# grasingerm/polymer-stats

Hardware: NVIDIA B200
Metric: monomer MC updates/sec (whole box), interacting n=512 dielectric chains (higher is better)
Workload: dtype f64

## Files before the change

polymer-stats_b200/csrc/cta_kernels.cuh:

```cuda
#pragma once

#include <type_traits>

#include "chain_math.cuh"

namespace pmc {

constexpr int kPartDoubles = 96;
constexpr int kRowDoubles = 26;

struct CtaView {
  double *sx, *sy, *sz;
  double *mx, *my, *mz;
  double *E;
  double *part;
  double *rowbuf;
  Proposal* prop;
  ChainDyn* dyn;
  ChainParams* par;
};

__host__ __device__ inline size_t cta_smem_bytes(int n) {
  size_t b = (size_t)7 * n * sizeof(double);
  b += (kPartDoubles + kRowDoubles) * sizeof(double);
// ... 101 lines not shown
    S.mx[i] = ux; S.my[i] = uy; S.mz[i] = uz;
  }
  team_sync<T>();
}

template <int T>
__device__ double cta_pair_energy(const CtaView& S, int n, int energy_type, double crad2 = 0.0) {
  constexpr int W = T / 32;
  const int tid = threadIdx.x, lane = tid & 31, warp = tid >> 5;
  double acc = 0.0;
  if (energy_type == 3) {
    for (int i = warp; i < n - 1; i += W) {
      const double xi = S.sx[i], yi = S.sy[i], zi = S.sz[i];
      const double ax = S.mx[i], ay = S.my[i], az = S.mz[i];
      for (int j = i + 1 + lane; j < n; j += 32)
        acc += pair_g_cut(ax, ay, az, S.mx[j], S.my[j], S.mz[j], xi - S.sx[j], yi - S.sy[j], zi - S.sz[j], crad2);
    }
  } else if (energy_type == 1) {
    for (int i = warp; i < n - 1; i += W) {
      const double xi = S.sx[i], yi = S.sy[i], zi = S.sz[i];
      const double ax = S.mx[i], ay = S.my[i], az = S.mz[i];
      for (int j = i + 1 + lane; j < n; j += 32)
        acc += pair_g(ax, ay, az, S.mx[j], S.my[j], S.mz[j], xi - S.sx[j], yi - S.sy[j], zi - S.sz[j]);
    }
  } else if (energy_type == 2) {
    for (int i = tid; i < n - 1; i += T)
      acc += pair_g(S.mx[i], S.my[i], S.mz[i], S.mx[i + 1], S.my[i + 1], S.mz[i + 1],
                    S.sx[i] - S.sx[i + 1], S.sy[i] - S.sy[i + 1], S.sz[i] - S.sz[i + 1]);
  }
  return block_sum<T>(acc, S.part);
}

template <int NW>
struct Team {
  static constexpr int kWarps = NW;
  static constexpr int kThreads = NW * 32;
  static constexpr int kLocalThreads = NW * 32;
  __device__ __forceinline__ static int tid() { return (int)threadIdx.x; }
  __device__ __forceinline__ static int ltid() { return tid(); }
  __device__ __forceinline__ static int warp() { return (int)(threadIdx.x >> 5); }
  __device__ __forceinline__ static int lane() { return (int)(threadIdx.x & 31); }
  __device__ __forceinline__ static void sync() { __syncthreads(); }
};

struct WarpTeam {
  static constexpr int kWarps = 1;
  static constexpr int kThreads = 32;
  static constexpr int kLocalThreads = 32;
  __device__ __forceinline__ static int tid() { return (int)(threadIdx.x & 31); }
  __device__ __forceinline__ static int ltid() { return tid(); }
  __device__ __forceinline__ static int warp() { return 0; }
  __device__ __forceinline__ static int lane() { return (int)(threadIdx.x & 31); }
  __device__ __forceinline__ static void sync() { __syncwarp(); }
};

struct LaneItem {
  double x, y, z;
  double ax, ay, az;
  double tx, ty, tz;
  double c;
  double w;
};

__device__ __forceinline__ LaneItem load_lane_item(const CtaView& S, int L, double Dx, double Dy, double Dz) {
  LaneItem it;
  it.x = S.sx[L]; it.y = S.sy[L]; it.z = S.sz[L];
  it.ax = S.mx[L]; it.ay = S.my[L]; it.az = S.mz[L];
  it.tx = -3.0 * it.ax; it.ty = -3.0 * it.ay; it.tz = -3.0 * it.az;
  it.c = fma(it.tz, Dz, fma(it.ty, Dy, it.tx * Dx));
  it.w = 0.0;
  return it;
}

__device__ __forceinline__ double rect_proj(double x, double y, double z, double px, double py, double pz, double Dx,
                                            double Dy, double Dz) {
  return fma(z - pz, Dz, fma(y - py, Dy, (x - px) * Dx));
}

__device__ __forceinline__ void rect_lane_w(LaneItem& it, double px, double py, double pz, double Dx, double Dy,
                                            double Dz) {
  it.w = -2.0 * rect_proj(it.x, it.y, it.z, px, py, pz, Dx, Dy, Dz);
}

template <bool Q2>
__device__ __forceinline__ void rect_prepass_item(const CtaView& S, int baseB, int k, double px, double py, double pz,
                                                  double Dx, double Dy, double Dz) {
  const int j = baseB + k;
  const double e = fma(S.mz[j], Dz, fma(S.my[j], Dy, S.mx[j] * Dx));
  if constexpr (Q2) {
    const double dd = fma(Dz, Dz, fma(Dy, Dy, Dx * Dx));
    reinterpret_cast<double2*>(S.E)[k] =
        make_double2(e, fma(2.0, rect_proj(S.sx[j], S.sy[j], S.sz[j], px, py, pz, Dx, Dy, Dz), dd));
  }
  else
    S.E[j] = e;
}

template <bool CUT = false, bool Q2 = false>
__device__ __forceinline__ double rect_pair(const LaneItem& it, double bx, double by, double bz, double ux,
                                            double uy, double uz, double e, double p2, double Dx, double Dy, double Dz,
                                            double acc, double crad2 = 0.0) {
  const double rx = it.x - bx, ry = it.y - by, rz = it.z - bz;
  const double mm = fma(it.az, uz, fma(it.ay, uy, it.ax * ux));
  const double r2 = fma(rz, rz, fma(ry, ry, rx * rx));
  const double a3 = fma(it.tz, rz, fma(it.ty, ry, it.tx * rx));
  const double bb = fma(uz, rz, fma(uy, ry, ux * rx));
  double q2;
  if constexpr (Q2) {
    q2 = (r2 + it.w) + p2;
  } else {
    const double qx = rx - Dx, qy = ry - Dy, qz = rz - Dz;
    q2 = fma(qz, qz, fma(qy, qy, qx * qx));
  }
  const double a3n = a3 - it.c;
  const double bn = bb - e;
  const double y = rsqrt_fast(r2);
  const double yn = rsqrt_fast(q2);
  const double y2 = y * y, yn2 = yn * yn;
  const double t = fma(a3 * bb, y2, mm);
  const double tn = fma(a3n * bn, yn2, mm);
  if constexpr (CUT) {
    const double gn = tn * (yn2 * yn), go = t * (y2 * y);
    return acc + ((q2 > crad2 ? 0.0 : gn) - (r2 > crad2 ? 0.0 : go));
  } else {
    acc = fma(tn, yn2 * yn, acc);
    return fma(-t, y2 * y, acc);
  }
}

template <class TEAM, int UNROLL = 2, bool CUT = false, bool EFLY = false, bool Q2 = false>
__device__ __forceinline__ double rect_sum(const CtaView& S, int baseA, int A, int baseB, int B, double Dx,
                                           double Dy, double Dz, double crad2 = 0.0, int pivot = 0) {
  static_assert(!(Q2 && EFLY), "the Q2 form reads 2p_B from the pre-pass");
  constexpr int W = TEAM::kWarps;
  const int lane = TEAM::lane(), warp = TEAM::warp();
  const int G = (A + 31) >> 5;
  const double* __restrict__ bxp = S.sx + baseB;
  const double* __restrict__ byp = S.sy + baseB;
  const double* __restrict__ bzp = S.sz + baseB;
  const double* __restrict__ mxp = S.mx + baseB;
  const double* __restrict__ myp = S.my + baseB;
  const double* __restrict__ mzp = S.mz + baseB;
  const double* __restrict__ ep = S.E + baseB;
  const double2* __restrict__ e2p = reinterpret_cast<const double2*>(S.E);
  auto lane_item = [&](int L) {
    LaneItem it = load_lane_item(S, L, Dx, Dy, Dz);
    if (Q2) {
      rect_lane_w(it, S.sx[pivot], S.sy[pivot], S.sz[pivot], Dx, Dy, Dz);
      asm("" : "+d"(it.tx), "+d"(it.ty), "+d"(it.tz));
    }
    return it;
  };
  auto bvals = [&](int k, double ux, double uy, double uz, double& e, double& p2) {
    if constexpr (Q2) {
      const double2 v = e2p[k];
      e = v.x; p2 = v.y;
    } else {
      e = EFLY ? fma(uz, Dz, fma(uy, Dy, ux * Dx)) : ep[k];
      p2 = 0.0;
    }
  };
  double acc = 0.0;
  const int G2 = G >> 1;
  {
    const int U = G2 * B;
    int u = (int)(((long long)U * warp) / W);
    const int u1 = (int)(((long long)U * (warp + 1)) / W);
    if (u < u1) {
      int g = u / B;
      int k = u - g * B;
      while (u < u1) {
        const int l0 = g * 64 + lane, l1 = l0 + 32;
        const bool v0 = l0 < A, v1 = l1 < A;
        const LaneItem i0 = lane_item(baseA + min(l0, A - 1));
        const LaneItem i1 = lane_item(baseA + min(l1, A - 1));
        const int kend = min(B, k + (u1 - u));
        u += kend - k;
        double a0 = 0.0, a1 = 0.0;
#pragma unroll UNROLL
        for (; k < kend; ++k) {
          const double bx = bxp[k], by = byp[k], bz = bzp[k];
          const double ux = mxp[k], uy = myp[k], uz = mzp[k];
          double e, p2;
          bvals(k, ux, uy, uz, e, p2);
          a0 = rect_pair<CUT, Q2>(i0, bx, by, bz, ux, uy, uz, e, p2, Dx, Dy, Dz, a0, crad2);
          a1 = rect_pair<CUT, Q2>(i1, bx, by, bz, ux, uy, uz, e, p2, Dx, Dy, Dz, a1, crad2);
        }
        acc += (v0 ? a0 : 0.0) + (v1 ? a1 : 0.0);
        k = 0;
        ++g;
      }
    }
  }
  if (G & 1) {
    int k = (int)(((long long)B * warp) / W);
    const int kend = (int)(((long long)B * (warp + 1)) / W);
    if (k < kend) {
      const int li = (G - 1) * 32 + lane;
      const bool valid = li < A;
      const LaneItem it = lane_item(baseA + min(li, A - 1));
      double a0 = 0.0, a1 = 0.0;
      auto pair = [&](int kk, double a) {
        double e, p2;
        bvals(kk, mxp[kk], myp[kk], mzp[kk], e, p2);
        return rect_pair<CUT, Q2>(it, bxp[kk], byp[kk], bzp[kk], mxp[kk], myp[kk], mzp[kk], e, p2, Dx, Dy, Dz, a,
                                  crad2);
      };
      for (; k + 1 < kend; k += 2) {
        a0 = pair(k, a0);
        a1 = pair(k + 1, a1);
      }
      if (k < kend) a0 = pair(k, a0);
      acc += valid ? (a0 + a1) : 0.0;
    }
  }
  return acc;
}

template <class TEAM, int UNROLL = 2>
__device__ __forceinline__ double delta_pairs_partial(const CtaView& S, int n, int energy_type, double b, int idx,
                                                      double npx, double npy, double npz,
                                                      double dnx, double dny, double dnz) {
  constexpr int T = TEAM::kThreads;
  const int tid = TEAM::tid();
  const double Dx = b * dnx, Dy = b * dny, Dz = b * dnz;
  const double hx = 0.5 * Dx, hy = 0.5 * Dy, hz = 0.5 * Dz;
  const int H = idx, Tl = n - 1 - idx;
  bool rect = (energy_type == 1) && H > 0 && Tl > 0;
  bool lanes_are_heads = true;
  if (rect) {
    const long long costH = (long long)((H + 31) >> 5) * Tl;
    const long long costT = (long long)((Tl + 31) >> 5) * H;
    lanes_are_heads = costH <= costT;
    if (2 * (lanes_are_heads ? Tl : H) > n) lanes_are_heads = !lanes_are_heads;
  }
  const double sgn = lanes_are_heads ? 1.0 : -1.0;
  const double ex = sgn * Dx, ey = sgn * Dy, ez = sgn * Dz;
  const int baseA = lanes_are_heads ? 0 : idx + 1, A = lanes_are_heads ? H : Tl;
  const int baseB = lanes_are_heads ? idx + 1 : 0, B = lanes_are_heads ? Tl : H;
  const double xi = S.sx[idx], yi = S.sy[idx], zi = S.sz[idx];
  if (rect)
    for (int k = TEAM::ltid(); k < B; k += TEAM::kLocalThreads)
      rect_prepass_item<true>(S, baseB, k, xi, yi, zi, ex, ey, ez);
  double acc = 0.0;
  {
    const double ox = S.mx[idx], oy = S.my[idx], oz = S.mz[idx];
    int jlo = 0, jhi = n - 1;
    if (energy_type == 2) { jlo = max(0, idx - 1); jhi = min(n - 1, idx + 1); }
    if (energy_type == 0) { jlo = 1; jhi = 0; }
    for (int j = jlo + tid; j <= jhi; j += T) {
      if (j == idx) continue;
      const double rx = xi - S.sx[j], ry = yi - S.sy[j], rz = zi - S.sz[j];
      const double s = (j < idx) ? 1.0 : -1.0;
      const double ux = S.mx[j], uy = S.my[j], uz = S.mz[j];
      acc += pair_g(npx, npy, npz, ux, uy, uz, fma(s, hx, rx), fma(s, hy, ry), fma(s, hz, rz)) -
             pair_g(ox, oy, oz, ux, uy, uz, rx, ry, rz);
    }
  }
  TEAM::sync();
  if (rect) acc += rect_sum<TEAM, UNROLL, false, false, true>(S, baseA, A, baseB, B, ex, ey, ez, 0.0, idx);
  return acc;
}

template <int T, int UNROLL = 2>
__device__ __forceinline__ double cta_delta_pairs(const CtaView& S, int n, int energy_type, double b, int idx,
                                                  double npx, double npy, double npz, double dnx, double dny,
                                                  double dnz) {
  const double acc = delta_pairs_partial<Team<T / 32>, UNROLL>(S, n, energy_type, b, idx, npx, npy, npz, dnx, dny, dnz);
  return block_sum<T>(acc, S.part, false);
}

}

#define PMC_CTA_BUILDING_BLOCKS 1
#include "cta_f32.cuh"

namespace pmc {

struct RunArgs {
  MonoRec* mono;
  const ChainParams* par;
  ChainDyn* dyn;
  double* traj;
  double* roll;
  long long nsteps, stepout, rows;
  uint64_t seed;
  uint32_t chain_id_base;
  int n;
  int nchains;
  int energy_type;
  ChainDynX* dynx;
  double* state;
  int roll_cols;
  int compensated;
  int window;
};

__device__ __forceinline__ void make_proposal(const RunArgs& a, const ChainParams& P, const ChainDyn& D,
                                              const MonoRec* mono, uint32_t chain_id, uint32_t init, long long step,
                                              Proposal& q) {
  const Draws d = draw_step(a.seed, chain_id, init, step, a.n);
  const MonoRec rec = mono[d.idx];
  double dphi, dtheta;
  increments(P, d, rec.theta, D.phi_step, D.theta_step, dphi, dtheta);
  build_proposal(P, rec, d.idx, dphi, dtheta, d.eps, q);
}

__device__ __forceinline__ void apply_decision(const ChainParams& P, ChainDyn& D, const Proposal& q, bool accept,
                                               double dU_pairs, long long step) {
  if (accept) {
    D.U += q.du + q.drF + dU_pairs;
    D.Omega += q.dOmega;
    D.su += q.du;
    D.r[0] += P.b * q.dnx; D.r[1] += P.b * q.dny; D.r[2] += P.b * q.dnz;
    D.p[0] += q.dmx; D.p[1] += q.dmy; D.p[2] += q.dmz;
    D.nacc += 1;
    D.nacc_total += 1;
  }
  D.natt += 1;
  D.steps_total += 1;
  D.step = step;
}

template <bool COMP = true>
__device__ __forceinline__ void bookkeep(const ChainParams& P, ChainDyn& D, long long step) {
  adapt_steps(P, step, D.phi_step, D.theta_step, D.nacc, D.natt);
  record_averages<COMP>(P, D.acc, D.comp, D.r, D.p, D.U, D.su, D.log_gauge);
}

template <bool COMP = true>
__device__ __forceinline__ void after_decision(const ChainParams& P, ChainDyn& D, const Proposal& q, bool accept,
                                               double dU_pairs, long long step) {
  apply_decision(P, D, q, accept, dU_pairs, step);
  bookkeep<COMP>(P, D, step);
}

__device__ __forceinline__ void stage_row(const ChainDyn& D, long long step, double* rowbuf) {
  rowbuf[0] = (double)step;
  rowbuf[1] = D.r[0]; rowbuf[2] = D.r[1]; rowbuf[3] = D.r[2];
  rowbuf[4] = D.p[0]; rowbuf[5] = D.p[1]; rowbuf[6] = D.p[2];
  rowbuf[7] = D.U;
  rowbuf[8] = (double)step;
  const double nrm = D.acc[16] + D.comp[16];
#pragma unroll
  for (int k = 0; k < 16; ++k) rowbuf[9 + k] = (D.acc[k] + D.comp[k]) / nrm;
}

__device__ __forceinline__ void emit_row(const RunArgs& a, const ChainDyn& D, int c, long long row, long long step,
                                         double* rowbuf, int tid) {
  if (tid == 0) stage_row(D, step, rowbuf);
  __syncwarp();
  if (row < a.rows) {
    if (tid < 8) a.traj[((size_t)c * a.rows + row) * 8 + tid] = rowbuf[tid];
    if (tid < 17) a.roll[((size_t)c * a.rows + row) * 17 + tid] = rowbuf[8 + tid];
  }
  __syncwarp();
}

__device__ __forceinline__ MonoRec record_of(const Proposal& q) {
  MonoRec rec;
  rec.phi = q.phi; rec.theta = q.theta;
  rec.nx = q.nx; rec.ny = q.ny; rec.nz = q.nz; rec.sth = q.sth;
  return rec;
}

__device__ __forceinline__ void shift_tail(const CtaView& S, int first, int n, double Dx, double Dy, double Dz, int tid,
                                           int stride) {
  for (int j = first + tid; j < n; j += stride) {
    S.sx[j] += Dx; S.sy[j] += Dy; S.sz[j] += Dz;
  }
}

__device__ __forceinline__ void move_pivot(const CtaView& S, MonoRec* mono, const Proposal& q, int idx, double b,
                                           double dnx, double dny, double dnz) {
  S.sx[idx] += 0.5 * b * dnx; S.sy[idx] += 0.5 * b * dny; S.sz[idx] += 0.5 * b * dnz;
  S.mx[idx] = q.mx; S.my[idx] = q.my; S.mz[idx] = q.mz;
  mono[idx] = record_of(q);
}

__device__ __forceinline__ bool decide(double single, double tsum, double inv_kT, double eps, double& dsum) {
  dsum = __dmul_rn(kInv4Pi, tsum);
  return metropolis(__fma_rn(-dsum, inv_kT, single), eps);
}

constexpr int kWin = 32;

__device__ __forceinline__ int window_len(const RunArgs& a, const ChainParams& P, bool adapt_on, long long step0,
                                          long long s, long long& to_boundary) {
  long long wl = a.nsteps - s + 1;
  if (wl > kWin) wl = kWin;
  to_boundary = 0;
  if (adapt_on) {
    to_boundary = P.steps_per_adjust - ((step0 + s - 1) % P.steps_per_adjust);
    if (wl > to_boundary) wl = to_boundary;
  }
  return (int)wl;
}

template <class Make>
__device__ __forceinline__ void build_window(long long step, int wlen, unsigned& dirty, int tid, Make&& make) {
  if (tid < wlen) make(tid, step + tid);
  if (tid == 0) dirty = 0u;
}

template <class Entry>
__device__ __forceinline__ void mark_stale(const Entry* win, int k, int wlen, int lo, int hi, unsigned& dirty,
                                           int tid) {
  const int widx = win[tid].idx;
  const bool stale = tid > k && tid < wlen && widx >= lo && widx <= hi;
  const unsigned m = __ballot_sync(0xffffffffu, stale);
  if (tid == 0 && m) dirty |= m;
}

__host__ __device__ inline size_t cta_smem_bytes_win(int n) {
  return (cta_smem_bytes(n) + kWin * sizeof(Proposal) + 16 + 15) & ~(size_t)15;
}
__host__ __device__ inline size_t cta_smem_bytes_win_f32(int n) { return cta_smem_bytes_win(n) + f32_smem_bytes(n); }

template <int T, int MINB, int UNROLL = 2, int PREC = 0>
__global__ void __launch_bounds__(T, MINB) k_run_cta_win(const RunArgs a) {
  extern __shared__ __align__(16) unsigned char smem_raw[];
  const CtaView S = carve(smem_raw, a.n);
  Proposal* win = reinterpret_cast<Proposal*>(smem_raw + cta_smem_bytes(a.n));
  unsigned* dirty = reinterpret_cast<unsigned*>(win + kWin);
  const F32View F = carve_f32(smem_raw + cta_smem_bytes_win(a.n), PREC ? a.n : 0, S.E);
  const int c = blockIdx.x;
  const int tid = threadIdx.x;
  const int n = a.n;
  MonoRec* mono = a.mono + (size_t)c * n;
  if (tid == 0) {
    *S.par = a.par[c];
    *S.dyn = a.dyn[c];
  }
  __syncthreads();
  const ChainParams& P = *S.par;
  load_chain<T>(mono, P, n, S);
  if (PREC) fill_mu_f32<Team<T / 32>>(S, F, n);
  const uint32_t chain_id = a.chain_id_base + (uint32_t)c;
  const double b = P.b, inv_kT = P.inv_kT;
  const long long step0 = S.dyn->step;
  const uint32_t init = (uint32_t)S.dyn->init;
  const bool adapt_on = P.adj_scale != 1.0 && P.steps_per_adjust > 0;
  long long row = 0;

  long long s = 1;
  while (s <= a.nsteps) {
    long long to_boundary;
    const int wlen = window_len(a, P, adapt_on, step0, s, to_boundary);
    if (tid < 32)
      build_window(step0 + s, wlen, *dirty, tid,
                   [&](int e, long long st) { make_proposal(a, P, *S.dyn, mono, chain_id, init, st, win[e]); });
    __syncthreads();
    for (int k = 0; k < wlen; ++k) {
      const long long step = step0 + s + k;
      if ((*dirty >> k) & 1u) {
        if (tid == 0) make_proposal(a, P, *S.dyn, mono, chain_id, (uint32_t)S.dyn->init, step, win[k]);
        __syncthreads();
      }
      const Proposal* q = &win[k];
      const int idx = q->idx;
      const bool skip = q->skip;
      const double dnx = q->dnx, dny = q->dny, dnz = q->dnz;
      double dsum = 0.0;
      bool accept = false;
      if (!skip) {
        const double t = PREC ? cta_delta_pairs_f32<T>(S, F, n, b, idx, q->mx, q->my, q->mz, dnx, dny, dnz)
                              : cta_delta_pairs<T, UNROLL>(S, n, 1, b, idx, q->mx, q->my, q->mz, dnx, dny, dnz);
        accept = decide(q->single, t, inv_kT, q->eps, dsum);
      }
      if (accept) {
        shift_tail(S, idx + 1, n, b * dnx, b * dny, b * dnz, tid, T);
        if (tid < 32) mark_stale(win, k, wlen, idx, idx, *dirty, tid);
      }
      if (tid == 0) {
        if (accept) {
          move_pivot(S, mono, *q, idx, b, dnx, dny, dnz);
          if (PREC) F.pb[idx] = make_float4((float)q->mx, (float)q->my, (float)q->mz, 0.0f);
        }
        after_decision(P, *S.dyn, *q, accept, dsum, step);
      }
      const bool isrow = a.stepout > 0 && (step % a.stepout) == 0;
      if (isrow && tid < 32) emit_row(a, *S.dyn, c, row, step, S.rowbuf, tid);
      if (isrow) ++row;
      __syncthreads();
    }
    s += wlen;
  }
  if (tid == 0) a.dyn[c] = *S.dyn;
}

struct SpecTrial {
  double dsum;
  int accept, pad;
};

__host__ __device__ inline int spec_e_stride(int n) { return (n + 1) & ~1; }

__host__ __device__ inline size_t cta_smem_bytes_spec(int n, int groups) {
  return cta_smem_bytes_win(n) +
         (((size_t)(groups - 1) * spec_e_stride(n) * sizeof(double) + (size_t)groups * sizeof(SpecTrial) + 15) & ~(size_t)15);
}

template <int G, int MINB>
__global__ void __launch_bounds__(32 * G, MINB) k_run_cta_win_spec(const RunArgs a) {
  constexpr int T = 32 * G;
  extern __shared__ __align__(16) unsigned char smem_raw[];
  const CtaView S = carve(smem_raw, a.n);
  Proposal* win = reinterpret_cast<Proposal*>(smem_raw + cta_smem_bytes(a.n));
  unsigned* dirty = reinterpret_cast<unsigned*>(win + kWin);
  double* extraE = reinterpret_cast<double*>(smem_raw + cta_smem_bytes_win(a.n));
  SpecTrial* res = reinterpret_cast<SpecTrial*>(extraE + (size_t)(G - 1) * spec_e_stride(a.n));
  const int c = blockIdx.x;
  const int tid = threadIdx.x, lane = tid & 31, g = tid >> 5;
  const int n = a.n;
  MonoRec* mono = a.mono + (size_t)c * n;
  CtaView Sg = S;
  if (g > 0) Sg.E = extraE + (size_t)(g - 1) * spec_e_stride(n);
  if (tid == 0) {
    *S.par = a.par[c];
    *S.dyn = a.dyn[c];
  }
  __syncthreads();
  const ChainParams& P = *S.par;
  load_chain<T>(mono, P, n, S);
  const uint32_t chain_id = a.chain_id_base + (uint32_t)c;
  const double b = P.b, inv_kT = P.inv_kT;
  const long long step0 = S.dyn->step;
  const uint32_t init = (uint32_t)S.dyn->init;
  const bool adapt_on = P.adj_scale != 1.0 && P.steps_per_adjust > 0;
  long long row = 0;
  Countdown row_due;
  row_due.start(step0, a.stepout);

  long long s = 1;
  while (s <= a.nsteps) {
    long long to_boundary;
    const int wlen = window_len(a, P, adapt_on, step0, s, to_boundary);
    if (tid < 32)
      build_window(step0 + s, wlen, *dirty, tid,
                   [&](int e, long long st) { make_proposal(a, P, *S.dyn, mono, chain_id, init, st, win[e]); });
    __syncthreads();
    int k = 0;
    while (k < wlen) {
      const int nb = min(G, wlen - k);
      if (g < nb) {
        const int kk = k + g;
        if ((*dirty >> kk) & 1u) {
          if (lane == 0) make_proposal(a, P, *S.dyn, mono, chain_id, (uint32_t)S.dyn->init, step0 + s + kk, win[kk]);
          __syncwarp();
        }
        const Proposal* q = &win[kk];
        double dsum = 0.0;
        bool accept = false;
// ... 225 lines not shown
```

polymer-stats_b200/csrc/plan.cu:

```cuda
#include "handle.h"

namespace {

constexpr size_t kSmemPerSm = 233472;

int64_t shape_chains(const pmc_handle* h) { return h->shape_chains > 0 ? h->shape_chains : h->nchains; }

int pick_cta_threads(int n) { return n <= 128 ? 64 : n <= 1024 ? 128 : n <= 1536 ? 256 : 512; }

int cluster_fit128(int n) {
  const int fit = (int)((size_t)kSmemMax / (pmc::cluster_smem_bytes(n, 128) + 1024));
  for (int mb : kCluster128Minb)
    if (fit >= mb) return mb;
  return kCluster128Minb[2];
}

int cluster_minb(int threads, int n) {
  if (threads == 32) return kTeamMinb[n <= 40 ? 0 : n <= 110 ? 1 : 2];
  return threads == 64 ? kCluster64Minb : threads == 128 ? cluster_fit128(n) : kCluster256Minb;
}

int scaled_threads(int base, int minb, size_t smem, int tmax, int64_t chains, int sms, int max_scale = 4) {
  const int fit = (int)std::max<size_t>(1, kSmemPerSm / (smem + 1024));
  const int resident_max = std::min(minb, fit);
// ... 6 lines not shown

int cta_block(const pmc_handle* h, int64_t chains) {
  const int base = pick_cta_threads(h->n);
  return scaled_threads(base, win_minb(base), pmc::cta_smem_bytes_win(h->n), 512, chains, h->sm_count);
}

template <class Smem, class Minb, class Fits>
int spec_teams(int64_t chains, int sms, int tries, Smem smem, Minb minb, Fits fits) {
  const int teams[3] = {8, 4, 2};
  for (int k = 0; k < tries; ++k) {
    const int fit = (int)std::min<size_t>((size_t)minb(teams[k]), kSmemPerSm / (smem(teams[k]) + 1024));
    if (fit >= 1 && chains <= (int64_t)sms * fit && fits(teams[k])) return teams[k];
  }
  return 0;
}

void plan_cluster_cta(const pmc_handle* h, int64_t chains, RunPlan& p) {
  const int n = h->n, base = pick_cluster_threads(n);
  auto delta_fits = [&](int t) { return pmc::cluster_delta_smem_bytes(n, t) <= (size_t)kSmemMax; };
  if (base == 32 && env_int("PMC_CLUSTER_SPEC", 1) != 0) {
    p.teams = spec_teams(chains, h->sm_count, 3, [&](int g) { return pmc::cluster_spec_smem_bytes(n, g); },
                         cluster_spec_minb, [&](int g) { return delta_fits(32 * g); });
    p.cta_threads = p.teams ? 32 * p.teams : 32;
  } else {
    p.cta_threads = scaled_threads(base, cluster_minb(base, n), pmc::cluster_smem_bytes(n, base), 256, chains, h->sm_count);
    while (p.cta_threads > base && !delta_fits(p.cta_threads)) p.cta_threads /= 2;
  }
  p.cut = h->energy_type == PMC_ENERGY_CUTOFF;
  p.threads = p.cta_threads;
  if (p.teams) {
    p.family = RunFamily::cta_cluster_spec;
    p.minb = cluster_spec_minb(p.teams);
    p.smem = pmc::cluster_spec_smem_bytes(n, p.teams);
  } else {
    p.family = RunFamily::cta_cluster;
    p.minb = cluster_minb(p.threads, n);
    p.smem = pmc::cluster_smem_bytes(n, p.threads);
  }
}

bool use_pair_kernel(int n, int threads, int64_t chains, int sms, int mode) {
  if (threads != 128 && threads != 256 && threads != 512) return false;
  if (pmc::cta_smem_bytes_win(n) > (size_t)kSmemMax) return true;
  if (mode == 0) return false;
  if (mode == 2) return true;
  if (pmc::cta_smem_bytes(n) > (size_t)kSmemMax / 2) return true;
  if (n > 768) return true;
  if (n > 384) {
    const double fill = (double)chains / ((double)sms * win_minb(threads));
    return fill >= 0.55 && fill < 0.9;
  }
  return false;
}

void plan_cta(const pmc_handle* h, int64_t chains, RunPlan& p) {
  const int n = h->n;
  p.threads = p.cta_threads;
  const int pair_mode = env_int("PMC_RUN_PAIR", 1);
  if (n <= 110 && h->pair_precision == PMC_PAIR_FP64 && pair_mode != 2 && env_int("PMC_RUN_SPEC", 1) != 0) {
    p.teams = spec_teams(chains, h->sm_count, n <= 64 ? 3 : 1, [&](int g) { return pmc::cta_smem_bytes_spec(n, g); },
                         spec_minb, [](int) { return true; });
    if (p.teams) {
      p.family = RunFamily::cta_win_spec;
      p.threads = 32 * p.teams;
      p.minb = spec_minb(p.teams);
      p.smem = pmc::cta_smem_bytes_spec(n, p.teams);
      return;
    }
  }
  if (use_pair_kernel(n, p.threads, chains, h->sm_count, pair_mode)) {
    p.family = RunFamily::cta_pair;
    p.smem = pmc::cta_smem_bytes(n);
    const int fit = (int)((size_t)kSmemMax / (p.smem + 1024)), cap = win_minb(p.threads);
    p.minb = std::max(1, std::min(fit, cap));
    const int o = env_int("PMC_PAIR_MINB", 0);
    if (o >= 1 && o <= cap) p.minb = o;
    p.pair_order = h->nchains <= 16384 && env_int("PMC_PAIR_ORDER", 1) != 0;
    return;
  }
  p.family = RunFamily::cta_win;
  p.minb = win_minb(p.threads);
  p.f32 = h->pair_precision == PMC_PAIR_FP32 && pmc::cta_smem_bytes_win_f32(n) <= (size_t)kSmemMax;
  p.smem = p.f32 ? pmc::cta_smem_bytes_win_f32(n) : pmc::cta_smem_bytes_win(n);
}

constexpr int64_t kWarpBelowIsing = 65536, kWarpBelowNonint = 120000;
void plan_lane(const pmc_handle* h, int64_t chains, RunPlan& p) {
  const int mode = env_int("PMC_LANE_MODE", 0);
  const int64_t below = p.ising ? kWarpBelowIsing : kWarpBelowNonint;
  if (mode == 2 || (mode == 0 && chains < below)) {
    p.family = RunFamily::warp;
    p.cpb = chains <= (int64_t)h->sm_count * 16 ? 1 : 4;
    p.threads = 32 * p.cpb;
    p.minb = warp_minb(p.cpb);
  } else {
    p.family = RunFamily::lane;
    p.threads = 64;
    p.minb = lane_minb(p.comp);
  }
}

constexpr int64_t kWarpClusterBelow = 11000, kLaneClusterMany = 32768;
void plan_lane_cluster(const pmc_handle* h, int64_t chains, RunPlan& p) {
  const int mode = env_int("PMC_LANE_CLUSTER_MODE", 0);
  if (mode == 2 || (mode == 0 && chains < kWarpClusterBelow)) {
    p.family = RunFamily::warp_cluster;
    p.threads = 128;
    p.minb = kWarpClusterMinb;
    p.stage = h->n <= kWarpClusterStageMax;
    p.smem = p.stage ? (size_t)4 * h->n * sizeof(MonoRec) : 0;
  } else {
    p.family = RunFamily::lane_cluster;
    p.threads = 64;
    p.minb = !p.comp && chains >= kLaneClusterMany ? kLaneClusterManyMinb : kLaneClusterMinb;
  }
}

}

RunPlan plan_run(const pmc_handle* h) {
  RunPlan p;
  const int64_t chains = shape_chains(h);
  p.cta_threads = cta_block(h, chains);
  p.ising = h->energy_type == PMC_ENERGY_ISING;
  p.comp = h->compensated != 0;
  const bool pair_sum = h->energy_type == PMC_ENERGY_INTERACTING || h->energy_type == PMC_ENERGY_CUTOFF;
  if (h->cluster_mode && pair_sum) plan_cluster_cta(h, chains, p);
  else if (h->cluster_mode) plan_lane_cluster(h, chains, p);
  else if (h->energy_type == PMC_ENERGY_INTERACTING) plan_cta(h, chains, p);
  else plan_lane(h, chains, p);
  return p;
}

std::string kernel_name(const RunPlan& p) {
  char b[96];
  const char* comp = p.comp ? "true" : "false";
  switch (p.family) {
    case RunFamily::cta_win:
      std::snprintf(b, sizeof b, "k_run_cta_win<%d,%d,%d%s>", p.threads, p.minb, kRunUnroll, p.f32 ? ",fp32" : ""); break;
    case RunFamily::cta_win_spec: std::snprintf(b, sizeof b, "k_run_cta_win_spec<%d,%d>", p.teams, p.minb); break;
    case RunFamily::cta_pair: std::snprintf(b, sizeof b, "k_run_cta_pair<%d,%d,%d>", p.threads, p.minb, kRunUnroll); break;
    case RunFamily::lane: std::snprintf(b, sizeof b, "k_run_lane<%d,%d,%s>", p.threads, p.minb, comp); break;
    case RunFamily::warp:
      std::snprintf(b, sizeof b, p.cpb == 1 ? "k_run_warp<%d,%d,%s,1>" : "k_run_warp<%d,%d,%s>", (int)p.ising, p.minb, comp);
      break;
    case RunFamily::cta_cluster:
      std::snprintf(b, sizeof b, "k_run_cta_cluster<%d,%d%s>", p.threads, p.minb, p.cut ? ",cut" : ""); break;
    case RunFamily::cta_cluster_spec:
      std::snprintf(b, sizeof b, "k_run_cta_cluster_spec<%d,%d%s>", p.teams, p.minb, p.cut ? ",cut" : ""); break;
    case RunFamily::lane_cluster:
      std::snprintf(b, sizeof b, "k_run_lane_cluster<%d,%d%s>", p.threads, p.minb, p.comp ? ",comp" : ""); break;
    case RunFamily::warp_cluster:
      std::snprintf(b, sizeof b, "k_run_warp_cluster<%s,%d,%s>", p.ising ? "true" : "false", p.minb, comp); break;
  }
  return b;
}
```

polymer-stats_b200/csrc/plan.h:

```cpp
#pragma once

#include <cstddef>
#include <string>

struct pmc_handle;

enum class RunFamily {
  cta_win,
  cta_win_spec,
  cta_pair,
  lane,
  warp,
  cta_cluster,
  cta_cluster_spec,
  lane_cluster,
  warp_cluster,
};

struct RunPlan {
  RunFamily family = RunFamily::cta_win;
  int threads = 0;
  int minb = 0;
  int teams = 0;
  int cpb = 0;
  bool f32 = false;
  bool cut = false;
  bool ising = false;
  bool comp = false;
  bool stage = false;
  bool pair_order = false;
  size_t smem = 0;
  int cta_threads = 0;
};

RunPlan plan_run(const pmc_handle* h);
std::string kernel_name(const RunPlan& p);

constexpr int kRunUnroll = 2;

constexpr int win_minb(int threads) { return 512 / threads; }
constexpr int spec_minb(int teams) { return teams == 8 ? 1 : teams == 4 ? 3 : 6; }
constexpr int cluster_spec_minb(int teams) { return teams == 8 ? 1 : teams == 4 ? 3 : 5; }
constexpr int kTeamMinb[3] = {16, 10, 8};
constexpr int kCluster64Minb = 5, kCluster128Minb[3] = {4, 3, 2}, kCluster256Minb = 1;
constexpr int warp_minb(int cpb) { return 16 / cpb; }
constexpr int lane_minb(bool comp) { return comp ? 4 : 6; }
constexpr int kLaneClusterMinb = 4, kLaneClusterManyMinb = 8;
constexpr int kWarpClusterMinb = 2;
```

polymer-stats_b200/csrc/run_cta.cu:

```cuda
#include "handle.h"

int launch_run_cta(pmc_handle* h, const RunPlan& p, const RunArgs& a) {
  const unsigned nb = (unsigned)h->nchains;
  if (p.family == RunFamily::cta_win_spec)
    return with<8, 4, 2>(p.teams, [&](auto G) {
      return launch(h, k_run_cta_win_spec<G, spec_minb(G)>, nb, p.threads, p.smem, a);
    });
  return with<64, 128, 256, 512>(p.threads, [&](auto T) {
    return p.f32 ? launch(h, k_run_cta_win<T, win_minb(T), kRunUnroll, 1>, nb, T, p.smem, a)
                 : launch(h, k_run_cta_win<T, win_minb(T), kRunUnroll, 0>, nb, T, p.smem, a);
  });
}
```

Measured before the change: 8.246 million.

## Cache per-bond rectangle energies so rejected moves compute only new-side pairs

```diff
diff --git a/polymer-stats_b200/csrc/cta_kernels.cuh b/polymer-stats_b200/csrc/cta_kernels.cuh
--- a/polymer-stats_b200/csrc/cta_kernels.cuh
+++ b/polymer-stats_b200/csrc/cta_kernels.cuh
@@ -253,10 +253,24 @@
   }
 }
 
-template <class TEAM, int UNROLL = 2, bool CUT = false, bool EFLY = false, bool Q2 = false>
+__device__ __forceinline__ double rect_pair_new(const LaneItem& it, double bx, double by, double bz, double ux,
+                                                double uy, double uz, double acc) {
+  const double rx = it.x - bx, ry = it.y - by, rz = it.z - bz;
+  const double mm = fma(it.az, uz, fma(it.ay, uy, it.ax * ux));
+  const double r2 = fma(rz, rz, fma(ry, ry, rx * rx));
+  const double a3 = fma(it.tz, rz, fma(it.ty, ry, it.tx * rx));
+  const double bb = fma(uz, rz, fma(uy, ry, ux * rx));
+  const double y = rsqrt_fast(r2);
+  const double y2 = y * y;
+  const double t = fma(a3 * bb, y2, mm);
+  return fma(t, y2 * y, acc);
+}
+
+template <class TEAM, int UNROLL = 2, bool CUT = false, bool EFLY = false, bool Q2 = false, bool NEW = false>
 __device__ __forceinline__ double rect_sum(const CtaView& S, int baseA, int A, int baseB, int B, double Dx,
                                            double Dy, double Dz, double crad2 = 0.0, int pivot = 0) {
   static_assert(!(Q2 && EFLY), "the Q2 form reads 2p_B from the pre-pass");
+  static_assert(!(NEW && (Q2 || EFLY || CUT)), "the new-only form reads nothing but the staged chain");
   constexpr int W = TEAM::kWarps;
   const int lane = TEAM::lane(), warp = TEAM::warp();
   const int G = (A + 31) >> 5;
@@ -270,6 +284,7 @@
   const double2* __restrict__ e2p = reinterpret_cast<const double2*>(S.E);
   auto lane_item = [&](int L) {
     LaneItem it = load_lane_item(S, L, Dx, Dy, Dz);
+    if (NEW) { it.x -= Dx; it.y -= Dy; it.z -= Dz; }
     if (Q2) {
       rect_lane_w(it, S.sx[pivot], S.sy[pivot], S.sz[pivot], Dx, Dy, Dz);
       asm("" : "+d"(it.tx), "+d"(it.ty), "+d"(it.tz));
@@ -306,10 +321,15 @@
         for (; k < kend; ++k) {
           const double bx = bxp[k], by = byp[k], bz = bzp[k];
           const double ux = mxp[k], uy = myp[k], uz = mzp[k];
-          double e, p2;
-          bvals(k, ux, uy, uz, e, p2);
-          a0 = rect_pair<CUT, Q2>(i0, bx, by, bz, ux, uy, uz, e, p2, Dx, Dy, Dz, a0, crad2);
-          a1 = rect_pair<CUT, Q2>(i1, bx, by, bz, ux, uy, uz, e, p2, Dx, Dy, Dz, a1, crad2);
+          double e = 0.0, p2 = 0.0;
+          if constexpr (!NEW) bvals(k, ux, uy, uz, e, p2);
+          if constexpr (NEW) {
+            a0 = rect_pair_new(i0, bx, by, bz, ux, uy, uz, a0);
+            a1 = rect_pair_new(i1, bx, by, bz, ux, uy, uz, a1);
+          } else {
+            a0 = rect_pair<CUT, Q2>(i0, bx, by, bz, ux, uy, uz, e, p2, Dx, Dy, Dz, a0, crad2);
+            a1 = rect_pair<CUT, Q2>(i1, bx, by, bz, ux, uy, uz, e, p2, Dx, Dy, Dz, a1, crad2);
+          }
         }
         acc += (v0 ? a0 : 0.0) + (v1 ? a1 : 0.0);
         k = 0;
@@ -326,6 +346,7 @@
       const LaneItem it = lane_item(baseA + min(li, A - 1));
       double a0 = 0.0, a1 = 0.0;
       auto pair = [&](int kk, double a) {
+        if constexpr (NEW) return rect_pair_new(it, bxp[kk], byp[kk], bzp[kk], mxp[kk], myp[kk], mzp[kk], a);
         double e, p2;
         bvals(kk, mxp[kk], myp[kk], mzp[kk], e, p2);
         return rect_pair<CUT, Q2>(it, bxp[kk], byp[kk], bzp[kk], mxp[kk], myp[kk], mzp[kk], e, p2, Dx, Dy, Dz, a,
@@ -342,6 +363,31 @@
   return acc;
 }
 
+struct RectSides {
+  bool rect;
+  double sgn;
+  int baseA, A, baseB, B;
+};
+
+__device__ __forceinline__ RectSides rect_sides(int n, int idx, bool pairs) {
+  const int H = idx, Tl = n - 1 - idx;
+  RectSides r;
+  r.rect = pairs && H > 0 && Tl > 0;
+  bool lanes_are_heads = true;
+  if (r.rect) {
+    const long long costH = (long long)((H + 31) >> 5) * Tl;
+    const long long costT = (long long)((Tl + 31) >> 5) * H;
+    lanes_are_heads = costH <= costT;
+    if (2 * (lanes_are_heads ? Tl : H) > n) lanes_are_heads = !lanes_are_heads;
+  }
+  r.sgn = lanes_are_heads ? 1.0 : -1.0;
+  r.baseA = lanes_are_heads ? 0 : idx + 1;
+  r.A = lanes_are_heads ? H : Tl;
+  r.baseB = lanes_are_heads ? idx + 1 : 0;
+  r.B = lanes_are_heads ? Tl : H;
+  return r;
+}
+
 template <class TEAM, int UNROLL = 2>
 __device__ __forceinline__ double delta_pairs_partial(const CtaView& S, int n, int energy_type, double b, int idx,
                                                       double npx, double npy, double npz,
@@ -350,19 +396,10 @@
   const int tid = TEAM::tid();
   const double Dx = b * dnx, Dy = b * dny, Dz = b * dnz;
   const double hx = 0.5 * Dx, hy = 0.5 * Dy, hz = 0.5 * Dz;
-  const int H = idx, Tl = n - 1 - idx;
-  bool rect = (energy_type == 1) && H > 0 && Tl > 0;
-  bool lanes_are_heads = true;
-  if (rect) {
-    const long long costH = (long long)((H + 31) >> 5) * Tl;
-    const long long costT = (long long)((Tl + 31) >> 5) * H;
-    lanes_are_heads = costH <= costT;
-    if (2 * (lanes_are_heads ? Tl : H) > n) lanes_are_heads = !lanes_are_heads;
-  }
-  const double sgn = lanes_are_heads ? 1.0 : -1.0;
-  const double ex = sgn * Dx, ey = sgn * Dy, ez = sgn * Dz;
-  const int baseA = lanes_are_heads ? 0 : idx + 1, A = lanes_are_heads ? H : Tl;
-  const int baseB = lanes_are_heads ? idx + 1 : 0, B = lanes_are_heads ? Tl : H;
+  const RectSides R = rect_sides(n, idx, energy_type == 1);
+  const bool rect = R.rect;
+  const double ex = R.sgn * Dx, ey = R.sgn * Dy, ez = R.sgn * Dz;
+  const int baseA = R.baseA, A = R.A, baseB = R.baseB, B = R.B;
   const double xi = S.sx[idx], yi = S.sy[idx], zi = S.sz[idx];
   if (rect)
     for (int k = TEAM::ltid(); k < B; k += TEAM::kLocalThreads)
@@ -395,6 +432,184 @@
   return block_sum<T>(acc, S.part, false);
 }
 
+constexpr double kRectCacheMaxAcc = 0.3;
+constexpr int kRectCacheMinTrials = 64;
+
+__host__ __device__ inline int rect_cache_bstride(int n) { return n / 2 + 1; }
+__host__ __device__ inline size_t rect_cache_bytes(int n, int threads) {
+  return ((size_t)2 * n + (size_t)(threads / 32) * rect_cache_bstride(n)) * sizeof(double);
+}
+
+struct RectCache {
+  double *R, *HT, *BP;
+};
+
+__device__ __forceinline__ RectCache carve_rect_cache(unsigned char* base, int n) {
+  RectCache C;
+  C.R = reinterpret_cast<double*>(base);
+  C.HT = C.R + n;
+  C.BP = C.HT + n;
+  return C;
+}
+
+template <class V, class Out>
+__device__ __forceinline__ void warp_scan_excl(int len, int lane, V&& v, Out&& out) {
+  const int C = (len + 31) >> 5;
+  const int t0 = min(len, lane * C), t1 = min(len, t0 + C);
+  double s = 0.0, c = 0.0;
+  for (int t = t0; t < t1; ++t) comp_add(s, c, v(t));
+  double is = s, ic = c;
+#pragma unroll
+  for (int o = 1; o < 32; o <<= 1) {
+    const double ts = __shfl_up_sync(0xffffffffu, is, o), tc = __shfl_up_sync(0xffffffffu, ic, o);
+    if (lane >= o) { comp_add(is, ic, ts); ic += tc; }
+  }
+  double ps = __shfl_up_sync(0xffffffffu, is, 1), pc = __shfl_up_sync(0xffffffffu, ic, 1);
+  if (lane == 0) { ps = 0.0; pc = 0.0; }
+  for (int t = t0; t < t1; ++t) {
+    out(t, ps + pc);
+    comp_add(ps, pc, v(t));
+  }
+}
+
+template <int T>
+__device__ void rect_cache_build(const CtaView& S, int n, const RectCache& C) {
+  const int tid = threadIdx.x;
+  for (int j = tid; j < n; j += T) {
+    const double xj = S.sx[j], yj = S.sy[j], zj = S.sz[j];
+    const double ax = S.mx[j], ay = S.my[j], az = S.mz[j];
+    double f = 0.0, g = 0.0;
+    for (int i = 0; i < n; ++i) {
+      const double u = pair_g(ax, ay, az, S.mx[i], S.my[i], S.mz[i], xj - S.sx[i], yj - S.sy[i], zj - S.sz[i]);
+      if (i > j) f += u;
+      else if (i < j) g += u;
+    }
+    C.HT[j] = f - g;
+    C.R[j] = g;
+  }
+  __syncthreads();
+  if (tid < 32)
+    warp_scan_excl(n, tid, [&](int t) { return C.HT[t]; }, [&](int t, double p) { C.R[t] = p - C.R[t]; });
+  __syncthreads();
+}
+
+template <int T, int UNROLL = 2>
+__device__ __forceinline__ void cta_delta_pairs_new(const CtaView& S, const RectCache& C, int n, double b, int idx,
+                                                    double npx, double npy, double npz, double dnx, double dny,
+                                                    double dnz, double& row, double& rnew, double& rold) {
+  constexpr int W = T / 32;
+  const int tid = threadIdx.x, lane = tid & 31, warp = tid >> 5;
+  const double Dx = b * dnx, Dy = b * dny, Dz = b * dnz;
+  const double hx = 0.5 * Dx, hy = 0.5 * Dy, hz = 0.5 * Dz;
+  const RectSides R = rect_sides(n, idx, true);
+  const double xi = S.sx[idx], yi = S.sy[idx], zi = S.sz[idx];
+  const double ox = S.mx[idx], oy = S.my[idx], oz = S.mz[idx];
+  rold = C.R[idx];
+  double acc = 0.0;
+  for (int j = tid; j < n; j += T) {
+    if (j == idx) continue;
+    const double rx = xi - S.sx[j], ry = yi - S.sy[j], rz = zi - S.sz[j];
+    const double s = (j < idx) ? 1.0 : -1.0;
+    const double ux = S.mx[j], uy = S.my[j], uz = S.mz[j];
+    const double d = pair_g(npx, npy, npz, ux, uy, uz, fma(s, hx, rx), fma(s, hy, ry), fma(s, hz, rz)) -
+                     pair_g(ox, oy, oz, ux, uy, uz, rx, ry, rz);
+    C.HT[j] = d;
+    acc += d;
+  }
+  double rn = 0.0;
+  if (R.rect)
+    rn = rect_sum<Team<W>, UNROLL, false, false, false, true>(S, R.baseA, R.A, R.baseB, R.B, R.sgn * Dx, R.sgn * Dy,
+                                                                R.sgn * Dz);
+  acc = warp_sum(acc);
+  rn = warp_sum(rn);
+  if (lane == 0) { S.part[warp] = acc; S.part[W + warp] = rn; }
+  __syncthreads();
+  row = 0.0; rnew = 0.0;
+#pragma unroll
+  for (int w = 0; w < W; ++w) { row += S.part[w]; rnew += S.part[W + w]; }
+}
+
+__device__ __forceinline__ double warp_sum4(double v0, double v1, double v2, double v3, int lane) {
+  const bool hi = (lane >> 4) & 1, c = (lane >> 3) & 1;
+  double a = hi ? v2 : v0, b = hi ? v3 : v1;
+  a += __shfl_xor_sync(0xffffffffu, hi ? v0 : v2, 16);
+  b += __shfl_xor_sync(0xffffffffu, hi ? v1 : v3, 16);
+  double x = c ? b : a;
+  x += __shfl_xor_sync(0xffffffffu, c ? a : b, 8);
+#pragma unroll
+  for (int o = 4; o > 0; o >>= 1) x += __shfl_xor_sync(0xffffffffu, x, o);
+  return x;
+}
+
+template <int T>
+__device__ void rect_cache_commit(const CtaView& S, const RectCache& C, int n, double b, int idx, double dnx, double dny,
+                                  double dnz, double rnew) {
+  constexpr int W = T / 32;
+  const int tid = threadIdx.x, lane = tid & 31, warp = tid >> 5;
+  const RectSides R = rect_sides(n, idx, true);
+  if (R.rect) {
+    const double ex = R.sgn * b * dnx, ey = R.sgn * b * dny, ez = R.sgn * b * dnz;
+    const double xi = S.sx[idx], yi = S.sy[idx], zi = S.sz[idx];
+    const int bstride = rect_cache_bstride(n);
+    double* __restrict__ bp = C.BP + warp * bstride;
+    for (int k = tid; k < R.B; k += T) rect_prepass_item<true>(S, R.baseB, k, xi, yi, zi, ex, ey, ez);
+    for (int k = lane; k < R.B; k += 32) bp[k] = 0.0;
+    __syncthreads();
+    const double* __restrict__ bxp = S.sx + R.baseB;
+    const double* __restrict__ byp = S.sy + R.baseB;
+    const double* __restrict__ bzp = S.sz + R.baseB;
+    const double* __restrict__ mxp = S.mx + R.baseB;
+    const double* __restrict__ myp = S.my + R.baseB;
+    const double* __restrict__ mzp = S.mz + R.baseB;
+    const double2* __restrict__ e2p = reinterpret_cast<const double2*>(S.E);
+    const int U = (R.A + 63) >> 6;
+    for (int u = warp; u < U; u += W) {
+      const int l0 = u * 64 + lane, l1 = l0 + 32;
+      const bool v0 = l0 < R.A, v1 = l1 < R.A;
+      LaneItem i0 = load_lane_item(S, R.baseA + min(l0, R.A - 1), ex, ey, ez);
+      LaneItem i1 = load_lane_item(S, R.baseA + min(l1, R.A - 1), ex, ey, ez);
+      rect_lane_w(i0, xi, yi, zi, ex, ey, ez);
+      rect_lane_w(i1, xi, yi, zi, ex, ey, ez);
+      double h0 = 0.0, h1 = 0.0;
+      for (int k0 = 0; k0 < R.B; k0 += 4) {
+        double s[4];
+#pragma unroll
+        for (int q = 0; q < 4; ++q) {
+          const bool kv = k0 + q < R.B;
+          const int k = kv ? k0 + q : R.B - 1;
+          const double2 e = e2p[k];
+          double d0 = rect_pair<false, true>(i0, bxp[k], byp[k], bzp[k], mxp[k], myp[k], mzp[k], e.x, e.y, ex, ey, ez, 0.0);
+          double d1 = rect_pair<false, true>(i1, bxp[k], byp[k], bzp[k], mxp[k], myp[k], mzp[k], e.x, e.y, ex, ey, ez, 0.0);
+          d0 = v0 && kv ? d0 : 0.0;
+          d1 = v1 && kv ? d1 : 0.0;
+          h0 += d0;
+          h1 += d1;
+          s[q] = d0 + d1;
+        }
+        const double t = warp_sum4(s[0], s[1], s[2], s[3], lane);
+        const int kq = k0 + (lane >> 3);
+        if ((lane & 7) == 0 && kq < R.B) bp[kq] += t;
+      }
+      if (v0) C.HT[R.baseA + l0] += h0;
+      if (v1) C.HT[R.baseA + l1] += h1;
+    }
+    __syncthreads();
+    for (int k = tid; k < R.B; k += T) {
+      double s = 0.0;
+#pragma unroll
+      for (int w = 0; w < W; ++w) s += C.BP[w * bstride + k];
+      C.HT[R.baseB + k] += s;
+    }
+    __syncthreads();
+  }
+  if (warp == 0)
+    warp_scan_excl(idx, lane, [&](int t) { return C.HT[t]; }, [&](int t, double p) { C.R[t] += p; });
+  else if (warp == 1)
+    warp_scan_excl(n - 1 - idx, lane, [&](int t) { return C.HT[n - 1 - t]; },
+                   [&](int t, double p) { C.R[n - 1 - t] += p; });
+  if (tid == 0) C.R[idx] = rnew;
+}
+
 }
 
 #define PMC_CTA_BUILDING_BLOCKS 1
@@ -419,6 +634,7 @@
   int roll_cols;
   int compensated;
   int window;
+  int rect_cache;
 };
 
 __device__ __forceinline__ void make_proposal(const RunArgs& a, const ChainParams& P, const ChainDyn& D,
@@ -549,6 +765,7 @@
   Proposal* win = reinterpret_cast<Proposal*>(smem_raw + cta_smem_bytes(a.n));
   unsigned* dirty = reinterpret_cast<unsigned*>(win + kWin);
   const F32View F = carve_f32(smem_raw + cta_smem_bytes_win(a.n), PREC ? a.n : 0, S.E);
+  const RectCache C = carve_rect_cache(smem_raw + cta_smem_bytes_win(a.n), a.n);
   const int c = blockIdx.x;
   const int tid = threadIdx.x;
   const int n = a.n;
@@ -561,6 +778,13 @@
   const ChainParams& P = *S.par;
   load_chain<T>(mono, P, n, S);
   if (PREC) fill_mu_f32<Team<T / 32>>(S, F, n);
+  bool cached = false;
+  if (!PREC && a.rect_cache) {
+    const ChainDyn& D0 = *S.dyn;
+    cached = a.rect_cache == 2 ||
+             (a.nsteps >= kRectCacheMinTrials && (double)D0.nacc_total <= kRectCacheMaxAcc * (double)D0.steps_total);
+    if (cached) rect_cache_build<T>(S, n, C);
+  }
   const uint32_t chain_id = a.chain_id_base + (uint32_t)c;
   const double b = P.b, inv_kT = P.inv_kT;
   const long long step0 = S.dyn->step;
@@ -586,14 +810,22 @@
       const int idx = q->idx;
       const bool skip = q->skip;
       const double dnx = q->dnx, dny = q->dny, dnz = q->dnz;
-      double dsum = 0.0;
+      double dsum = 0.0, rnew = 0.0;
       bool accept = false;
       if (!skip) {
-        const double t = PREC ? cta_delta_pairs_f32<T>(S, F, n, b, idx, q->mx, q->my, q->mz, dnx, dny, dnz)
-                              : cta_delta_pairs<T, UNROLL>(S, n, 1, b, idx, q->mx, q->my, q->mz, dnx, dny, dnz);
+        double t;
+        if (!PREC && cached) {
+          double row, rold;
+          cta_delta_pairs_new<T, UNROLL>(S, C, n, b, idx, q->mx, q->my, q->mz, dnx, dny, dnz, row, rnew, rold);
+          t = (rnew - rold) + row;
+        } else {
+          t = PREC ? cta_delta_pairs_f32<T>(S, F, n, b, idx, q->mx, q->my, q->mz, dnx, dny, dnz)
+                   : cta_delta_pairs<T, UNROLL>(S, n, 1, b, idx, q->mx, q->my, q->mz, dnx, dny, dnz);
+        }
         accept = decide(q->single, t, inv_kT, q->eps, dsum);
       }
       if (accept) {
+        if (!PREC && cached) rect_cache_commit<T>(S, C, n, b, idx, dnx, dny, dnz, rnew);
         shift_tail(S, idx + 1, n, b * dnx, b * dny, b * dnz, tid, T);
         if (tid < 32) mark_stale(win, k, wlen, idx, idx, *dirty, tid);
       }
diff --git a/polymer-stats_b200/csrc/plan.cu b/polymer-stats_b200/csrc/plan.cu
--- a/polymer-stats_b200/csrc/plan.cu
+++ b/polymer-stats_b200/csrc/plan.cu
@@ -112,6 +112,15 @@
   p.minb = win_minb(p.threads);
   p.f32 = h->pair_precision == PMC_PAIR_FP32 && pmc::cta_smem_bytes_win_f32(n) <= (size_t)kSmemMax;
   p.smem = p.f32 ? pmc::cta_smem_bytes_win_f32(n) : pmc::cta_smem_bytes_win(n);
+  const int rc = env_int("PMC_RECT_CACHE", 1);
+  if (!p.f32 && rc != 0) {
+    const size_t smem = p.smem + pmc::rect_cache_bytes(n, p.threads);
+    auto resident = [&](size_t b) { return std::min<size_t>(p.minb, kSmemPerSm / (b + 1024)); };
+    if (smem <= (size_t)kSmemMax && (rc == 2 || resident(smem) == resident(p.smem))) {
+      p.rect_cache = rc == 2 ? 2 : 1;
+      p.smem = smem;
+    }
+  }
 }
 
 constexpr int64_t kWarpBelowIsing = 65536, kWarpBelowNonint = 120000;
diff --git a/polymer-stats_b200/csrc/plan.h b/polymer-stats_b200/csrc/plan.h
--- a/polymer-stats_b200/csrc/plan.h
+++ b/polymer-stats_b200/csrc/plan.h
@@ -29,6 +29,7 @@
   bool comp = false;
   bool stage = false;
   bool pair_order = false;
+  int rect_cache = 0;
   size_t smem = 0;
   int cta_threads = 0;
 };
diff --git a/polymer-stats_b200/csrc/run_cta.cu b/polymer-stats_b200/csrc/run_cta.cu
--- a/polymer-stats_b200/csrc/run_cta.cu
+++ b/polymer-stats_b200/csrc/run_cta.cu
@@ -6,8 +6,10 @@
     return with<8, 4, 2>(p.teams, [&](auto G) {
       return launch(h, k_run_cta_win_spec<G, spec_minb(G)>, nb, p.threads, p.smem, a);
     });
+  RunArgs b = a;
+  b.rect_cache = p.rect_cache;
   return with<64, 128, 256, 512>(p.threads, [&](auto T) {
-    return p.f32 ? launch(h, k_run_cta_win<T, win_minb(T), kRunUnroll, 1>, nb, T, p.smem, a)
-                 : launch(h, k_run_cta_win<T, win_minb(T), kRunUnroll, 0>, nb, T, p.smem, a);
+    return p.f32 ? launch(h, k_run_cta_win<T, win_minb(T), kRunUnroll, 1>, nb, T, p.smem, b)
+                 : launch(h, k_run_cta_win<T, win_minb(T), kRunUnroll, 0>, nb, T, p.smem, b);
   });
 }
```

After: 10.70 million (median of 6 runs). 29.7% higher.

## Tile rectangular pair sum with transposed remainder strip to cut idle lanes

Applied to the files above, without the earlier changes.

```diff
diff --git a/polymer-stats_b200/csrc/cta_kernels.cuh b/polymer-stats_b200/csrc/cta_kernels.cuh
--- a/polymer-stats_b200/csrc/cta_kernels.cuh
+++ b/polymer-stats_b200/csrc/cta_kernels.cuh
@@ -207,18 +207,12 @@
   it.w = -2.0 * rect_proj(it.x, it.y, it.z, px, py, pz, Dx, Dy, Dz);
 }
 
-template <bool Q2>
-__device__ __forceinline__ void rect_prepass_item(const CtaView& S, int baseB, int k, double px, double py, double pz,
+__device__ __forceinline__ void rect_prepass_item(const CtaView& S, int j, int k, double px, double py, double pz,
                                                   double Dx, double Dy, double Dz) {
-  const int j = baseB + k;
   const double e = fma(S.mz[j], Dz, fma(S.my[j], Dy, S.mx[j] * Dx));
-  if constexpr (Q2) {
-    const double dd = fma(Dz, Dz, fma(Dy, Dy, Dx * Dx));
-    reinterpret_cast<double2*>(S.E)[k] =
-        make_double2(e, fma(2.0, rect_proj(S.sx[j], S.sy[j], S.sz[j], px, py, pz, Dx, Dy, Dz), dd));
-  }
-  else
-    S.E[j] = e;
+  const double dd = fma(Dz, Dz, fma(Dy, Dy, Dx * Dx));
+  reinterpret_cast<double2*>(S.E)[k] =
+      make_double2(e, fma(2.0, rect_proj(S.sx[j], S.sy[j], S.sz[j], px, py, pz, Dx, Dy, Dz), dd));
 }
 
 template <bool CUT = false, bool Q2 = false>
@@ -253,10 +247,9 @@
   }
 }
 
-template <class TEAM, int UNROLL = 2, bool CUT = false, bool EFLY = false, bool Q2 = false>
+template <class TEAM, int UNROLL = 2, bool CUT = false, bool EFLY = false>
 __device__ __forceinline__ double rect_sum(const CtaView& S, int baseA, int A, int baseB, int B, double Dx,
-                                           double Dy, double Dz, double crad2 = 0.0, int pivot = 0) {
-  static_assert(!(Q2 && EFLY), "the Q2 form reads 2p_B from the pre-pass");
+                                           double Dy, double Dz, double crad2 = 0.0) {
   constexpr int W = TEAM::kWarps;
   const int lane = TEAM::lane(), warp = TEAM::warp();
   const int G = (A + 31) >> 5;
@@ -267,23 +260,10 @@
   const double* __restrict__ myp = S.my + baseB;
   const double* __restrict__ mzp = S.mz + baseB;
   const double* __restrict__ ep = S.E + baseB;
-  const double2* __restrict__ e2p = reinterpret_cast<const double2*>(S.E);
-  auto lane_item = [&](int L) {
-    LaneItem it = load_lane_item(S, L, Dx, Dy, Dz);
-    if (Q2) {
-      rect_lane_w(it, S.sx[pivot], S.sy[pivot], S.sz[pivot], Dx, Dy, Dz);
-      asm("" : "+d"(it.tx), "+d"(it.ty), "+d"(it.tz));
-    }
-    return it;
-  };
+  auto lane_item = [&](int L) { return load_lane_item(S, L, Dx, Dy, Dz); };
   auto bvals = [&](int k, double ux, double uy, double uz, double& e, double& p2) {
-    if constexpr (Q2) {
-      const double2 v = e2p[k];
-      e = v.x; p2 = v.y;
-    } else {
-      e = EFLY ? fma(uz, Dz, fma(uy, Dy, ux * Dx)) : ep[k];
-      p2 = 0.0;
-    }
+    e = EFLY ? fma(uz, Dz, fma(uy, Dy, ux * Dx)) : ep[k];
+    p2 = 0.0;
   };
   double acc = 0.0;
   const int G2 = G >> 1;
@@ -308,8 +288,8 @@
           const double ux = mxp[k], uy = myp[k], uz = mzp[k];
           double e, p2;
           bvals(k, ux, uy, uz, e, p2);
-          a0 = rect_pair<CUT, Q2>(i0, bx, by, bz, ux, uy, uz, e, p2, Dx, Dy, Dz, a0, crad2);
-          a1 = rect_pair<CUT, Q2>(i1, bx, by, bz, ux, uy, uz, e, p2, Dx, Dy, Dz, a1, crad2);
+          a0 = rect_pair<CUT>(i0, bx, by, bz, ux, uy, uz, e, p2, Dx, Dy, Dz, a0, crad2);
+          a1 = rect_pair<CUT>(i1, bx, by, bz, ux, uy, uz, e, p2, Dx, Dy, Dz, a1, crad2);
         }
         acc += (v0 ? a0 : 0.0) + (v1 ? a1 : 0.0);
         k = 0;
@@ -328,8 +308,8 @@
       auto pair = [&](int kk, double a) {
         double e, p2;
         bvals(kk, mxp[kk], myp[kk], mzp[kk], e, p2);
-        return rect_pair<CUT, Q2>(it, bxp[kk], byp[kk], bzp[kk], mxp[kk], myp[kk], mzp[kk], e, p2, Dx, Dy, Dz, a,
-                                  crad2);
+        return rect_pair<CUT>(it, bxp[kk], byp[kk], bzp[kk], mxp[kk], myp[kk], mzp[kk], e, p2, Dx, Dy, Dz, a,
+                              crad2);
       };
       for (; k + 1 < kend; k += 2) {
         a0 = pair(k, a0);
@@ -338,6 +318,100 @@
       if (k < kend) a0 = pair(k, a0);
       acc += valid ? (a0 + a1) : 0.0;
     }
+  }
+  return acc;
+}
+
+struct RectTiling {
+  int baseA, A;
+  int baseB, B;
+  int At, Bc;
+  int V1, V;
+};
+
+__device__ __forceinline__ RectTiling rect_tiling(int n, int idx) {
+  RectTiling R;
+  const int H = idx, Tl = n - 1 - idx;
+  const bool lanes_are_heads = H >= Tl;
+  R.baseA = lanes_are_heads ? 0 : idx + 1; R.A = lanes_are_heads ? H : Tl;
+  R.baseB = lanes_are_heads ? idx + 1 : 0; R.B = lanes_are_heads ? Tl : H;
+  const int Ar = R.A & 63, Br = R.B & 63;
+  R.At = 2 * (R.B + Ar) <= n ? Ar : 0;
+  R.Bc = Br < R.At ? Br : 0;
+  R.V1 = ((R.A - R.At + 63) >> 6) * R.B + R.Bc;
+  R.V = R.V1 + ((R.B - R.Bc + 63) >> 6) * R.At;
+  return R;
+}
+
+__device__ __forceinline__ void rect_prepass(const CtaView& S, const RectTiling& R, double px, double py, double pz,
+                                             double Dx, double Dy, double Dz, int t, int stride) {
+  for (int k = t; k < R.B + R.At; k += stride) {
+    if (k < R.B) rect_prepass_item(S, R.baseB + k, k, px, py, pz, Dx, Dy, Dz);
+    else rect_prepass_item(S, R.baseA + R.A - R.At + (k - R.B), k, px, py, pz, -Dx, -Dy, -Dz);
+  }
+}
+
+template <class TEAM, int UNROLL = 2>
+__device__ __forceinline__ double rect_sum_q2(const CtaView& S, const RectTiling& R, double Dx, double Dy, double Dz,
+                                              int pivot) {
+  constexpr int W = TEAM::kWarps;
+  const int lane = TEAM::lane(), warp = TEAM::warp();
+  auto lane_item = [&](int L, double s) {
+    LaneItem it = load_lane_item(S, L, s * Dx, s * Dy, s * Dz);
+    rect_lane_w(it, S.sx[pivot], S.sy[pivot], S.sz[pivot], s * Dx, s * Dy, s * Dz);
+    asm("" : "+d"(it.tx), "+d"(it.ty), "+d"(it.tz));
+    return it;
+  };
+  double acc = 0.0;
+  const int GT = R.At ? (R.V - R.V1) / R.At : 0;
+  int m0 = 0, m1 = 0;
+#pragma unroll
+  for (int w2 = 0; w2 <= W; ++w2) {
+    if (w2 > warp + 1) break;
+    const long long cnt = (long long)w2 * (GT / W) + min(w2, GT % W);
+    const long long m = (long long)R.V * w2 / W - (long long)R.At * cnt;
+    const int mm = (int)max(0LL, min((long long)R.V1, m));
+    if (w2 <= warp) m0 = max(m0, mm);
+    m1 = max(m1, mm);
+  }
+  int jt = warp;
+  int u = m0, u1 = m1;
+  for (;;) {
+    if (u >= u1) {
+      if (jt >= GT) break;
+      u = R.V1 + jt * R.At; u1 = u + R.At; jt += W;
+    }
+    const bool tr = u >= R.V1;
+    const int v = tr ? u - R.V1 : u;
+    const int K = tr ? R.At : R.B;
+    const int lbase = tr ? R.baseB + R.Bc : R.baseA, nl = tr ? R.B - R.Bc : R.A;
+    const int bbase = tr ? R.baseA + R.A - R.At : R.baseB;
+    const double2* __restrict__ e2p = reinterpret_cast<const double2*>(S.E) + (tr ? R.B : 0);
+    const int g = v / K;
+    int k = v - g * K;
+    const int kend = min(K, k + (u1 - u));
+    u += kend - k;
+    const int l0 = g * 64 + lane, l1 = l0 + 32;
+    const bool v0 = l0 < nl, v1 = l1 < nl;
+    const double s = tr ? -1.0 : 1.0;
+    const LaneItem i0 = lane_item(lbase + min(l0, nl - 1), s);
+    const LaneItem i1 = lane_item(lbase + min(l1, nl - 1), s);
+    const double* __restrict__ bxp = S.sx + bbase;
+    const double* __restrict__ byp = S.sy + bbase;
+    const double* __restrict__ bzp = S.sz + bbase;
+    const double* __restrict__ mxp = S.mx + bbase;
+    const double* __restrict__ myp = S.my + bbase;
+    const double* __restrict__ mzp = S.mz + bbase;
+    double a0 = 0.0, a1 = 0.0;
+#pragma unroll UNROLL
+    for (; k < kend; ++k) {
+      const double bx = bxp[k], by = byp[k], bz = bzp[k];
+      const double ux = mxp[k], uy = myp[k], uz = mzp[k];
+      const double2 ev = e2p[k];
+      a0 = rect_pair<false, true>(i0, bx, by, bz, ux, uy, uz, ev.x, ev.y, Dx, Dy, Dz, a0);
+      a1 = rect_pair<false, true>(i1, bx, by, bz, ux, uy, uz, ev.x, ev.y, Dx, Dy, Dz, a1);
+    }
+    acc += (v0 ? a0 : 0.0) + (v1 ? a1 : 0.0);
   }
   return acc;
 }
@@ -350,23 +424,12 @@
   const int tid = TEAM::tid();
   const double Dx = b * dnx, Dy = b * dny, Dz = b * dnz;
   const double hx = 0.5 * Dx, hy = 0.5 * Dy, hz = 0.5 * Dz;
-  const int H = idx, Tl = n - 1 - idx;
-  bool rect = (energy_type == 1) && H > 0 && Tl > 0;
-  bool lanes_are_heads = true;
-  if (rect) {
-    const long long costH = (long long)((H + 31) >> 5) * Tl;
-    const long long costT = (long long)((Tl + 31) >> 5) * H;
-    lanes_are_heads = costH <= costT;
-    if (2 * (lanes_are_heads ? Tl : H) > n) lanes_are_heads = !lanes_are_heads;
-  }
-  const double sgn = lanes_are_heads ? 1.0 : -1.0;
+  const bool rect = (energy_type == 1) && idx > 0 && idx < n - 1;
+  const RectTiling R = rect_tiling(n, idx);
+  const double sgn = R.baseA == 0 ? 1.0 : -1.0;
   const double ex = sgn * Dx, ey = sgn * Dy, ez = sgn * Dz;
-  const int baseA = lanes_are_heads ? 0 : idx + 1, A = lanes_are_heads ? H : Tl;
-  const int baseB = lanes_are_heads ? idx + 1 : 0, B = lanes_are_heads ? Tl : H;
   const double xi = S.sx[idx], yi = S.sy[idx], zi = S.sz[idx];
-  if (rect)
-    for (int k = TEAM::ltid(); k < B; k += TEAM::kLocalThreads)
-      rect_prepass_item<true>(S, baseB, k, xi, yi, zi, ex, ey, ez);
+  if (rect) rect_prepass(S, R, xi, yi, zi, ex, ey, ez, TEAM::ltid(), TEAM::kLocalThreads);
   double acc = 0.0;
   {
     const double ox = S.mx[idx], oy = S.my[idx], oz = S.mz[idx];
@@ -383,7 +446,7 @@
     }
   }
   TEAM::sync();
-  if (rect) acc += rect_sum<TEAM, UNROLL, false, false, true>(S, baseA, A, baseB, B, ex, ey, ez, 0.0, idx);
+  if (rect) acc += rect_sum_q2<TEAM, UNROLL>(S, R, ex, ey, ez, idx);
   return acc;
 }
 
```

New measurement: 8.257 million before, 8.633 million after, median of 6. 4.6% higher.
